# openclimatefix/graph_weather

Measured on AMD Instinct MI355X. Metric: forward forecasts/sec (1° grid, 102→78 feat), higher is better.
Workload: dtype f32; 1 GPU; c2: GraphWeatherForecaster 1deg grid (64800 nodes), 102->78 feat, batch=2 on rank 0, fp32, mesh res 2 (5882 nodes), random-init weights; global_batch=2, parallelism=batch-sharded x1, no collective in forward

## Files before the change

graph_weather_amd/csrc/gw_internal.hpp:

```cpp
#ifndef GW_INTERNAL_HPP
#define GW_INTERNAL_HPP

#include <hip/hip_runtime_api.h>
#include <stdint.h>

#include "../../include/gw_amd.h"

namespace gw {

enum { EPI_ROWS = 0, EPI_EDGE = 1, EPI_DEC = 2 };

struct ChainArgs {
  int n_cols;
  int cols_per_batch;
  unsigned long long* dbg;
  int dbg_cap;
  int stagger;
  const float* seg_ptr[3];
  const int* seg_idx[3];
  int seg_rows_pb[3];
  int seg_ld[3];
  int seg_k[3];
  int seg_proj[3];
  int seg_half[3];
  int seg_bf16k[3];
  const float* proj_w[4];
  float* proj_out[4];
  int n_post;
  const float* hd_w1;
  const float* hd_b1;
  const float* hd_w2;
  const float* hd_b2;
  const float* hd_w3;
  const float* hd_b3;
  int tune16;
  int proj_half;
  const float* w1[3];
  const float* b1;
  const float* w_mid;
  const float* b_mid;
  const float* w_out;
  const float* b_out;
  const float* gamma;
  const float* beta;
  int n_mid;
  const float* res_ptr;
  const int* res_idx;
  int res_rows_pb;
  int res_ld;
  float* out;
  int out_ld;
  int out_cols;
  int ln_width;
  float* agg;
  const int* agg_idx;
  int agg_rows_pb;
  const float* relu_mask;
  float* zero_rows;
  float* carry;
  float* save_h;
  long long save_stride;
  int save_ld;
  float* save_y;
};

int chain16_launch(int kind, ChainArgs& a, int k_in, int hidden, int n_out, int grid_y, void* stream);
int chainx3_launch(int kind, ChainArgs& a, int k_in, int hidden, int n_out, int grid_y, void* stream);
struct BwdChainArgs {
  const float* d;
  const void* w[5];
  const float* mask[2];
  float* out[5];
  long long n_rows;
  int d_ld, n_chain, n_fan;
  const float* ln_y;
  const float* ln_gamma;
  float* ln_dgamma;
  float* ln_dbeta;
  float* ln_dy;
  const float* add[5];
  int add_ld;
  float* colsum;
  const int* d_idx;
  int d_idx_n, d_tab_rows_pb;
  const float* d_add;
  int d_add_ld;
  unsigned add_d_mask;
};
int bwd_chainx3_launch(const BwdChainArgs& a, void* stream);
void pack_x3_item(const float* w, long long stride_f, long long stride_k, int n_out, int kseg, int ntp, int nsteps, void* out, void* stream);

int node_rs_groups(int64_t n_cols);
bool node_rs_eligible(const ChainArgs& a);
int node_rs_launch(ChainArgs& a, bool x3 , void* stream);

extern unsigned long long* g_dbg;
extern int g_dbg_cap;
extern int g_dbg_kind;
#ifdef GW_TUNING
int env_int(const char* name, int fallback);
#define GW_TUNE(name, fallback) gw::env_int(name, fallback)
#define GW_SKIP(a) ((a).skip)
#define GW_TUNE_ARG(a) ((a).tune)
#else
#define GW_TUNE(name, fallback) (fallback)
#define GW_SKIP(a) 0
#define GW_TUNE_ARG(a) 0
#endif

struct DeviceOnce {
  bool done[64] = {};
  bool first() {
    int d = 0;
    if (hipGetDevice(&d) != hipSuccess || d < 0 || d >= 64) return true;
    if (done[d]) return false;
    done[d] = true;
    return true;
  }
};
int set_error(int code, const char* msg);
int check_launch(const char* what);

constexpr int kCarryFloats = 528;
size_t segment_carry_bytes(int64_t n_tiles);
int segment_fixup_launch(int64_t n_tiles, const float* carry, float* agg, void* stream);

bool edge_fast_eligible(const gw_operand* x_src, const gw_operand* x_dst, const gw_operand* e_in, const gw_mlp_weights* w);
int edge_fast_launch(int32_t batch, int32_t n_edges, const int32_t* src, const int32_t* dst, const gw_operand* x_src,
                     const gw_operand* x_dst, const gw_operand* e_in, const gw_operand* e_res, const gw_mlp_weights* w,
                     float* e_out, float* agg, int32_t n_dst, const gw_activation_save* save, float* carry ,
                     void* stream);
size_t edge_fast_carry_bytes(int32_t batch, int32_t n_edges);

bool edge_stream_eligible(const gw_operand* x_src, const gw_operand* x_dst, const gw_operand* e_in, const gw_mlp_weights* w);
int edge_stream_launch(int32_t batch, int32_t n_edges, const int32_t* src, const int32_t* dst, const gw_operand* x_src,
                       const gw_operand* x_dst, const gw_operand* e_in, const gw_mlp_weights* w, float* agg, int32_t n_dst,
                       void* stream);

bool edge16_eligible(const gw_operand* x_src, const gw_operand* x_dst, const gw_operand* e_in, const gw_mlp_weights* w);
size_t edge16_workspace_bytes(int32_t batch, int32_t n_edges);
int edge16_launch(int32_t batch, int32_t n_edges, const int32_t* src, const int32_t* dst, const gw_operand* x_src,
                  const gw_operand* x_dst, const gw_operand* e_in, const gw_operand* e_res, const gw_mlp_weights* w,
                  float* e_out, void* e_out_tiles, float* agg, int32_t n_dst, void* workspace, int32_t flags ,
                  void* stream);
size_t edge16_workspace_needed(int32_t batch, int32_t n_edges, const gw_operand* e_in, bool deterministic);
int edge16t_launch(const void* edge16_args , bool gather, int n_wg, void* stream);
int edge16p_launch(const void* edge16_args , int n_wg, void* stream);
int edge16_rows_to_tiles(int32_t batch, int32_t n_edges, const float* rows, int32_t rows_per_batch, int32_t ld, void* tiles,
                         void* stream);

int ln_bwd_wide_launch(int64_t rows, int32_t width, const float* dn, int32_t ld_dn, const float* y, int32_t ld_y, const float* gamma,
                       float* dy, int32_t ld_dy, float* dgamma, float* dbeta, void* stream);
int relu_mask_wide_launch(int64_t rows, int32_t width, const float* dh, int32_t ld_dh, const float* h, int32_t ld_h, float* dz,
                          int32_t ld_dz, float* db, void* stream);

}

#endif
```

graph_weather_amd/csrc/gw_kernels.hip:

```cpp

#include <hip/hip_runtime.h>
#include <stdint.h>
#include <stdio.h>
#include <stdlib.h>
#include <string.h>

#include "../../include/gw_amd.h"
#include "gw_device.hpp"
#include "gw_internal.hpp"

using namespace gw;

namespace {

template <int NSTEPS>
__device__ __forceinline__ void load_operand_slice(float (&in)[NSTEPS], const float* __restrict__ row, int c, int q) {
#pragma unroll
  for (int i = 2 * c; i < 2 * c + 2; ++i) {
    if (4 * i + 3 < NSTEPS) {
      const f32x4 v = ldg4(row + 16 * i + 4 * q);
      in[4 * i + 0] = v.x;
      in[4 * i + 1] = v.y;
      in[4 * i + 2] = v.z;
      in[4 * i + 3] = v.w;
// ... 927 lines not shown
    if (a.bf16) {
      a.nsteps[i] = m.kseg <= 32 ? 1 : (m.kseg <= 128 ? 4 : (m.kseg + 31) / 32);
      a.ntq[i] = (nt + 3) / 4 * 4;
    } else {
      a.nsteps[i] = packed_steps_f32(m.kseg);
      a.ntq[i] = (nt + 3) / 4;
    }
  }
  for (int i = 0; i < n_vecs; ++i) {
    if (!vecs[i].v || !vecs[i].out || vecs[i].n <= 0) return fail(GW_E_BADARG, "gw_pack_many: bad vector item");
    a.v[i] = vecs[i];
  }
  hipLaunchKernelGGL(pack_many_kernel, dim3(64, n_mats + (n_vecs > 0 ? 1 : 0)), dim3(256), 0, (hipStream_t)stream, a);
  return check_launch("pack_many_kernel launch");
}

namespace {
int fill_bwd_chain(BwdChainArgs& a, int64_t n_rows, const float* d, int32_t d_ld, int32_t n_chain, const void* const* chain_w,
                   const float* const* chain_mask, float* const* chain_out, int32_t n_fan, const void* const* fan_w, float* const* fan_out) {
  if (n_rows < 0 || !d || d_ld < 256 || d_ld % 4 != 0 || n_chain < 0 || n_chain > 2 || n_fan < 0 || n_fan > 3 || n_chain + n_fan < 1 ||
      (n_chain > 0 && (!chain_w || !chain_mask || !chain_out)) || (n_fan > 0 && (!fan_w || !fan_out)))
    return fail(GW_E_BADARG, "gw_mlp_chain_backward: bad arguments");
  memset(&a, 0, sizeof(a));
  a.d = d;
  a.d_ld = d_ld;
  a.n_rows = n_rows;
  a.n_chain = n_chain;
  a.n_fan = n_fan;
  for (int i = 0; i < n_chain; ++i) {
    if (!chain_w[i] || !chain_mask[i] || !chain_out[i]) return fail(GW_E_BADARG, "gw_mlp_chain_backward: NULL chain item");
    a.w[i] = chain_w[i];
    a.mask[i] = chain_mask[i];
    a.out[i] = chain_out[i];
  }
  for (int i = 0; i < n_fan; ++i) {
    if (!fan_w[i] || !fan_out[i]) return fail(GW_E_BADARG, "gw_mlp_chain_backward: NULL fan item");
    a.w[n_chain + i] = fan_w[i];
    a.out[n_chain + i] = fan_out[i];
  }
  if ((n_rows + kColsPerWG - 1) / kColsPerWG > 0x7fffffffLL) return fail(GW_E_BADARG, "gw_mlp_chain_backward: too many rows");
  return GW_OK;
}
}

int gw_mlp_chain_backward(int64_t n_rows, const float* d, int32_t d_ld, int32_t n_chain, const float* const* chain_w,
                          const float* const* chain_mask, float* const* chain_out, int32_t n_fan, const float* const* fan_w,
                          float* const* fan_out, void* stream) {
  BwdChainArgs a;
  if (int rc = fill_bwd_chain(a, n_rows, d, d_ld, n_chain, (const void* const*)chain_w, chain_mask, chain_out, n_fan, (const void* const*)fan_w,
                              fan_out))
    return rc;
  if (n_rows == 0) return GW_OK;
  return bwd_chain_launch(a, stream);
}

int gw_mlp_ln_chain_backward(int32_t weight_dtype, int64_t n_rows, const float* dn, int32_t dn_ld, const int32_t* dn_idx,
                             int32_t dn_idx_n, int32_t dn_table_rows_pb, const float* dn_add, int32_t dn_add_ld, const float* y,
                             const float* gamma, float* dgamma, float* dbeta, float* dy, int32_t n_chain, const void* const* chain_w,
                             const float* const* chain_mask, float* const* chain_out, float* dz_colsum, int32_t n_fan,
                             const void* const* fan_w, float* const* fan_out, const float* const* fan_add, int32_t fan_add_ld,
                             uint32_t fan_add_dn_mask, void* stream) {
  const bool ln = y != nullptr;
  if (ln && (!gamma || !dgamma || !dbeta || !dy)) return fail(GW_E_BADARG, "gw_mlp_ln_chain_backward: NULL LayerNorm argument");
  if (weight_dtype != GW_DTYPE_BF16X3 && weight_dtype != GW_DTYPE_F32)
    return fail(GW_E_UNSUPPORTED, "gw_mlp_ln_chain_backward: fp32 or split (GW_DTYPE_BF16X3) streams");
  if (dz_colsum && n_chain < 1) return fail(GW_E_BADARG, "gw_mlp_ln_chain_backward: dz_colsum needs a chain product");
  if (fan_add && (fan_add_ld < 256 || fan_add_ld % 4 != 0)) return fail(GW_E_BADARG, "gw_mlp_ln_chain_backward: bad fan_add_ld");
  if ((dn_idx || dn_add) && !ln) return fail(GW_E_UNSUPPORTED, "gw_mlp_ln_chain_backward: a gathered input gradient needs the LayerNorm in front");
  if (dn_add && !dn_idx) return fail(GW_E_BADARG, "gw_mlp_ln_chain_backward: dn_add goes with dn_idx");
  if (dn_idx && (dn_idx_n <= 0 || dn_table_rows_pb <= 0 || n_rows % dn_idx_n != 0 || (dn_add && (dn_add_ld < 256 || dn_add_ld % 4 != 0))))
    return fail(GW_E_BADARG, "gw_mlp_ln_chain_backward: bad gather arguments");
  if (fan_add_dn_mask >> (n_fan > 0 ? n_fan : 0)) return fail(GW_E_BADARG, "gw_mlp_ln_chain_backward: fan_add_dn_mask names a fan item that does not exist");
  BwdChainArgs a;
  if (int rc = fill_bwd_chain(a, n_rows, dn, dn_ld, n_chain, chain_w, chain_mask, chain_out, n_fan, fan_w, fan_out)) return rc;
  if (n_rows == 0) return GW_OK;
  if (ln) {
    a.ln_y = y;
    a.ln_gamma = gamma;
    a.ln_dgamma = dgamma;
    a.ln_dbeta = dbeta;
    a.ln_dy = dy;
  }
  a.d_idx = dn_idx;
  a.d_idx_n = dn_idx_n;
  a.d_tab_rows_pb = dn_table_rows_pb;
  a.d_add = dn_add;
  a.d_add_ld = dn_add_ld;
  a.colsum = dz_colsum;
  a.add_ld = fan_add_ld;
  for (int i = 0; fan_add && i < n_fan; ++i) a.add[n_chain + i] = fan_add[i];
  a.add_d_mask = fan_add_dn_mask << n_chain;
  return weight_dtype == GW_DTYPE_BF16X3 ? bwd_chainx3_launch(a, stream) : bwd_chain_launch(a, stream);
}

int gw_mlp_chain_backward_bf16x3(int64_t n_rows, const float* d, int32_t d_ld, int32_t n_chain, const void* const* chain_w,
                                 const float* const* chain_mask, float* const* chain_out, int32_t n_fan, const void* const* fan_w,
                                 float* const* fan_out, void* stream) {
  BwdChainArgs a;
  if (int rc = fill_bwd_chain(a, n_rows, d, d_ld, n_chain, chain_w, chain_mask, chain_out, n_fan, fan_w, fan_out)) return rc;
  if (n_rows == 0) return GW_OK;
  return bwd_chainx3_launch(a, stream);
}

int gw_pad_vector(const float* v, int n, float* out, void* stream) {
  if (!v || !out || n <= 0) return fail(GW_E_BADARG, "gw_pad_vector: bad arguments");
  const int npad = gw_padded_n(n);
  hipLaunchKernelGGL(pad_vector_kernel, dim3((npad + 255) / 256), dim3(256), 0, (hipStream_t)stream, v, n, npad, out);
  return check_launch("pad_vector_kernel launch");
}

namespace {
int fill_save(ChainArgs& a, const gw_activation_save* save, const gw_mlp_weights* w, const char* who) {
  if (!save) return GW_OK;
  if (w->weight_dtype == GW_DTYPE_BF16)
    return fail(GW_E_UNSUPPORTED, "activation saving (training) is implemented for fp32 and bf16x3 weights (the saves are fp32 rows)");
  if (!save->hidden || save->hidden_ld < w->hidden || save->hidden_ld % 4 != 0 || (w->ln_gamma && !save->pre_norm)) {
    snprintf(g_err, sizeof(g_err), "%s: bad gw_activation_save", who);
    return GW_E_BADARG;
  }
  a.save_h = save->hidden;
  a.save_stride = save->hidden_stride;
  a.save_ld = save->hidden_ld;
  a.save_y = save->pre_norm;
  return GW_OK;
}
}

int gw_mlp_forward(int64_t n_rows, int32_t rows_per_batch, const gw_operand* x, const gw_mlp_weights* w,
                   const gw_operand* residual, float* out, int32_t out_ld, const gw_activation_save* save, void* stream) {
  if (!x || !w || !out || n_rows < 0 || rows_per_batch <= 0) return fail(GW_E_BADARG, "gw_mlp_forward: bad arguments");
  if (n_rows == 0) return GW_OK;
  if (n_rows >= (int64_t)1 << 31) return fail(GW_E_UNSUPPORTED, "gw_mlp_forward: more than 2^31-1 rows");
  if (x->k <= 0 || !w->w1[0] || !w->w_out || !w->b1 || !w->b_out)
    return fail(GW_E_BADARG, "gw_mlp_forward: missing weights / empty operand");
  if (x->layout != GW_LAYOUT_ROWS_F32 || (residual && residual->layout != GW_LAYOUT_ROWS_F32))
    return fail(GW_E_UNSUPPORTED, "gw_mlp_forward: operands are fp32 rows");
  if (bad_layers(w)) return fail(GW_E_UNSUPPORTED, "gw_mlp_forward: at least 2 hidden layers (n_mid >= 1) are required");
  ChainArgs a;
  memset(&a, 0, sizeof(a));
  a.n_cols = (int)n_rows;
  a.cols_per_batch = rows_per_batch;
  fill_operand(a, 0, x);
  fill_weights(a, w);
  if (residual) {
    a.res_ptr = residual->ptr;
    a.res_idx = residual->index;
    a.res_rows_pb = residual->rows_per_batch;
    a.res_ld = residual->ld;
  }
  a.out = out;
  a.out_ld = out_ld;
  a.out_cols = w->n_out;
  if (int rc = fill_save(a, save, w, "gw_mlp_forward")) return rc;
  if (is16(w->weight_dtype)) {
    if (residual && w->n_out == 256 && (residual->ld % 4 != 0)) return fail(GW_E_UNSUPPORTED, "gw_mlp_forward: residual ld must be a multiple of 4");
    if (w->n_out == 256 && out_ld % 4 != 0) return fail(GW_E_UNSUPPORTED, "gw_mlp_forward: out_ld must be a multiple of 4");
    if (x->k == 256 && x->ld % 4 != 0) return fail(GW_E_UNSUPPORTED, "gw_mlp_forward: input ld must be a multiple of 4");
    if (x->k > 128 && x->k != 256) return fail(GW_E_UNSUPPORTED, "gw_mlp_forward: input width must be <=128 or ==256");
    if (w->weight_dtype == GW_DTYPE_BF16 && w->ln_gamma && (w->n_out != 256 || (w->ln_width > 0 && w->ln_width != w->n_out)))
      return fail(GW_E_UNSUPPORTED, "gw_mlp_forward: LayerNorm over fewer than 256 features is implemented for float32 and bf16x3 weights");
    return launch16(w->weight_dtype, 0, a, x->k, w->hidden, w->n_out, 1, stream);
  }
  if (w->hidden == 256 && w->n_out == 256) {
    if (residual && (residual->ld % 4 != 0)) return fail(GW_E_UNSUPPORTED, "gw_mlp_forward: residual ld must be a multiple of 4");
    if (out_ld % 4 != 0) return fail(GW_E_UNSUPPORTED, "gw_mlp_forward: out_ld must be a multiple of 4");
    if (x->k <= 16) return launch_chain(chain_kernel<4, false, 1, 16, 16, EPI_ROWS>, a, stream);
    if (x->k <= 112) return launch_chain(chain_kernel<28, false, 1, 16, 16, EPI_ROWS>, a, stream);
    if (x->k == 256 && x->ld % 4 == 0) return launch_chain(chain_kernel<64, true, 1, 16, 16, EPI_ROWS>, a, stream);
    return fail(GW_E_UNSUPPORTED, "gw_mlp_forward: input width must be <=112 or ==256 for hidden 256");
  }
  if (w->hidden == 256 && w->n_out <= 80 && x->k == 256 && x->ld % 4 == 0) {
    return launch_chain(chain_kernel<64, true, 1, 16, 5, EPI_DEC>, a, stream);
  }
  if (w->hidden == 128 && w->n_out <= 80 && x->k == 256 && x->ld % 4 == 0) {
    return launch_chain(chain_kernel<64, true, 1, 8, 5, EPI_DEC>, a, stream);
  }
  return fail(GW_E_UNSUPPORTED, "gw_mlp_forward: unsupported (hidden, n_out, k) combination");
}

int gw_mlp_post_forward(int64_t n_rows, int32_t rows_per_batch, const gw_operand* x, const gw_mlp_weights* w, float* out,
                        int32_t out_ld, int32_t n_post, const float* const* post_w, void* const* post_out, int32_t post_layout,
                        void* stream) {
  if (!x || !w || n_rows < 0 || rows_per_batch <= 0 || n_post <= 0 || n_post > 4 || !post_w || !post_out)
    return fail(GW_E_BADARG, "gw_mlp_post_forward: bad arguments");
  if (n_rows == 0) return GW_OK;
  if (n_rows >= (int64_t)1 << 31) return fail(GW_E_UNSUPPORTED, "gw_mlp_post_forward: more than 2^31-1 rows");
  if (x->k <= 0 || !w->w1[0] || !w->w_out || !w->b1 || !w->b_out) return fail(GW_E_BADARG, "gw_mlp_post_forward: missing weights / empty operand");
  if (x->layout != GW_LAYOUT_ROWS_F32) return fail(GW_E_UNSUPPORTED, "gw_mlp_post_forward: x is fp32 rows");
  if (bad_layers(w)) return fail(GW_E_UNSUPPORTED, "gw_mlp_post_forward: at least 2 hidden layers (n_mid >= 1) are required");
  if (!is16(w->weight_dtype) || w->hidden != 256 || w->n_out != 256 || !w->ln_gamma || (w->ln_width > 0 && w->ln_width != 256))
    return fail(GW_E_UNSUPPORTED, "gw_mlp_post_forward: bf16 / bf16x3 weights, hidden 256, 256 outputs with LayerNorm");
  if (post_layout != GW_LAYOUT_ROWS_F32 && post_layout != GW_LAYOUT_ROWS_F16) return fail(GW_E_BADARG, "gw_mlp_post_forward: bad post_layout");
  if (post_layout == GW_LAYOUT_ROWS_F16 && w->weight_dtype != GW_DTYPE_BF16)
    return fail(GW_E_UNSUPPORTED, "gw_mlp_post_forward: fp16 products come with bf16 weights");
  if (out && out_ld % 4 != 0) return fail(GW_E_UNSUPPORTED, "gw_mlp_post_forward: out_ld must be a multiple of 4");
  ChainArgs a;
  memset(&a, 0, sizeof(a));
  a.n_cols = (int)n_rows;
  a.cols_per_batch = rows_per_batch;
  fill_operand(a, 0, x);
  fill_weights(a, w);
  a.out = out;
  a.out_ld = out ? out_ld : 256;
  a.out_cols = 256;
  for (int i = 0; i < n_post; ++i) {
    if (!post_w[i] || !post_out[i]) return fail(GW_E_BADARG, "gw_mlp_post_forward: null post slice / output");
    a.proj_w[i] = post_w[i];
    a.proj_out[i] = (float*)post_out[i];
  }
  a.n_post = n_post;
  a.proj_half = post_layout == GW_LAYOUT_ROWS_F16;
  return launch16(w->weight_dtype, 5, a, x->k, w->hidden, w->n_out, 1, stream);
}

size_t gw_edge_update_workspace_bytes(int32_t batch, int32_t n_edges, const gw_operand* x_src, const gw_operand* x_dst,
                                      const gw_operand* e_in, const gw_mlp_weights* w, int32_t flags) {
  if (batch <= 0 || n_edges <= 0 || !x_src || !x_dst || !e_in || !w) return 0;
  const bool det = (flags & GW_EDGE_DETERMINISTIC) != 0;
  if (gw::edge16_eligible(x_src, x_dst, e_in, w)) return gw::edge16_workspace_needed(batch, n_edges, e_in, det);
  if (det && w->weight_dtype == GW_DTYPE_F32 && gw::edge_fast_eligible(x_src, x_dst, e_in, w)) return gw::edge_fast_carry_bytes(batch, n_edges);
  if (det && is16(w->weight_dtype)) return gw::edge_fast_carry_bytes(batch, n_edges);
  return 0;
}

size_t gw_edge_tiles_bytes(int32_t batch, int32_t n_edges) {
  if (batch <= 0 || n_edges <= 0) return 0;
  return gw::edge16_workspace_bytes(batch, n_edges);
}

int gw_edge_rows_to_tiles(int32_t batch, int32_t n_edges, const float* rows, int32_t rows_per_batch, int32_t ld, void* tiles,
                          void* stream) {
  if (batch <= 0 || n_edges <= 0 || !rows || !tiles || ld < 256 || ld % 4 != 0 || rows_per_batch < 0)
    return fail(GW_E_BADARG, "gw_edge_rows_to_tiles: bad arguments");
  return gw::edge16_rows_to_tiles(batch, n_edges, rows, rows_per_batch, ld, tiles, stream);
}

int gw_edge_update_forward(int32_t batch, int32_t n_edges, const int32_t* src, const int32_t* dst,
                           const gw_operand* x_src, const gw_operand* x_dst, const gw_operand* e_in,
                           const gw_operand* e_res, const gw_mlp_weights* w, void* e_out_any, int32_t e_out_layout, float* agg,
                           int32_t n_dst, const gw_activation_save* save, void* workspace, size_t workspace_bytes, int32_t flags,
                           void* stream) {
  if (batch <= 0 || n_edges < 0 || n_dst <= 0) return fail(GW_E_BADARG, "gw_edge_update_forward: bad arguments");
  if (n_edges == 0) return GW_OK;
  if (!src || !dst || !x_src || !x_dst || !e_in || !e_res || !w || !agg) return fail(GW_E_BADARG, "gw_edge_update_forward: bad arguments");
  if ((int64_t)batch * n_edges >= (int64_t)1 << 31 || (int64_t)batch * n_dst >= (int64_t)1 << 31)
    return fail(GW_E_UNSUPPORTED, "gw_edge_update_forward: batch*edges exceeds int32");
  if (w->hidden != 256 || w->n_out != 256 || (w->ln_gamma == nullptr) != (w->ln_beta == nullptr) || !w->b1 || !w->w_out || !w->b_out)
    return fail(GW_E_UNSUPPORTED, "gw_edge_update_forward: only hidden=256, out=256 is implemented");
  if (bad_layers(w)) return fail(GW_E_UNSUPPORTED, "gw_edge_update_forward: at least 2 hidden layers (n_mid >= 1) are required");
  const gw_operand* ops[3] = {x_src, x_dst, e_in};
  for (int i = 0; i < 3; ++i) {
    if (ops[i]->k == 0) continue;
    if (ops[i]->k != 256 || ops[i]->ld % 4 != 0 || !ops[i]->ptr || (!ops[i]->projected && !w->w1[i]))
      return fail(GW_E_UNSUPPORTED, "gw_edge_update_forward: operands must be 256 wide (or k=0 for zeros)");
  }
  const bool no_res = e_res->k == 0;
  const bool x3 = w->weight_dtype == GW_DTYPE_BF16X3;
  const bool stream32 = no_res && !(flags & (GW_EDGE_DETERMINISTIC | GW_EDGE_SEGMENT_TILES)) && gw::edge_stream_eligible(x_src, x_dst, e_in, w);
  if (no_res && (e_out_any != nullptr || save || !(x3 || stream32 || (gw::edge16_eligible(x_src, x_dst, e_in, w) && !(flags & GW_EDGE_DETERMINISTIC)))))
    return fail(GW_E_UNSUPPORTED, "gw_edge_update_forward: an edge update without residual (e_res.k == 0) is implemented for the bf16 "
                                  "path with resident weights (atomics mode), for bf16x3 weights and for float32 weights with projected "
                                  "operands only (one middle layer, LayerNorm over 256, atomics mode), without e_out or activation saving");
  if (!no_res && (e_res->k != 256 || e_res->ld % 4 != 0 || !e_res->ptr))
    return fail(GW_E_UNSUPPORTED, "gw_edge_update_forward: e_res (residual edge features) must be 256 wide");
  const bool tiles_in = (e_in->k > 0 && e_in->layout == GW_LAYOUT_EDGE_TILES_BF16) || e_res->layout == GW_LAYOUT_EDGE_TILES_BF16;
  const bool tiles_out = e_out_any != nullptr && e_out_layout == GW_LAYOUT_EDGE_TILES_BF16;
  if (e_out_any != nullptr && e_out_layout != GW_LAYOUT_ROWS_F32 && e_out_layout != GW_LAYOUT_EDGE_TILES_BF16)
    return fail(GW_E_BADARG, "gw_edge_update_forward: bad e_out_layout");
  if ((e_in->k > 0 && e_in->layout != GW_LAYOUT_ROWS_F32 && e_in->layout != GW_LAYOUT_EDGE_TILES_BF16) ||
      (!no_res && e_res->layout != GW_LAYOUT_ROWS_F32 && e_res->layout != GW_LAYOUT_EDGE_TILES_BF16))
    return fail(GW_E_UNSUPPORTED, "gw_edge_update_forward: edge operands are fp32 rows or bf16 edge tiles");
  const bool half_nodes = x_src->layout == GW_LAYOUT_ROWS_F16 || x_dst->layout == GW_LAYOUT_ROWS_F16;
  if ((x_src->layout != GW_LAYOUT_ROWS_F32 && x_src->layout != GW_LAYOUT_ROWS_F16) ||
      (x_dst->layout != GW_LAYOUT_ROWS_F32 && x_dst->layout != GW_LAYOUT_ROWS_F16) ||
      (half_nodes && (save || !gw::edge16_eligible(x_src, x_dst, e_in, w))))
    return fail(GW_E_UNSUPPORTED, "gw_edge_update_forward: node operands must be fp32 rows (or, projected, for the bf16 path with "
                                  "resident weights: fp16 product rows)");
  float* e_out = tiles_out ? nullptr : (float*)e_out_any;
  const bool det = (flags & GW_EDGE_DETERMINISTIC) != 0;
  const bool seg = (flags & GW_EDGE_SEGMENT_TILES) != 0;
  if ((flags & (GW_EDGE_AGG_BF16K | GW_EDGE_SEGMENT_SPLIT)) && !seg)
    return fail(GW_E_BADARG, "gw_edge_update_forward: GW_EDGE_AGG_BF16K / GW_EDGE_SEGMENT_SPLIT come with GW_EDGE_SEGMENT_TILES");
  if (seg) {
    const size_t ws_seg = gw::edge16_eligible(x_src, x_dst, e_in, w) ? gw::edge16_workspace_needed(batch, n_edges, e_in, false) : 0;
    if (det || save || n_edges % 64 != 0 || !gw::edge16_eligible(x_src, x_dst, e_in, w) || (e_out_any && !tiles_out) ||
        (!no_res && e_res->layout != GW_LAYOUT_EDGE_TILES_BF16) || (ws_seg > 0 && (!workspace || workspace_bytes < ws_seg)))
      return fail(GW_E_UNSUPPORTED, "gw_edge_update_forward: segment-aligned tiles (GW_EDGE_SEGMENT_TILES) are implemented for the bf16 "
                                    "path with resident weights: projected node operands, residual none or bf16 edge tiles, e' none "
                                    "or bf16 edge tiles, atomics mode, n_edges a multiple of 64, the workspace of "
                                    "gw_edge_update_workspace_bytes");
    return gw::edge16_launch(batch, n_edges, src, dst, x_src, x_dst, e_in, e_res, w, nullptr, tiles_out ? e_out_any : nullptr, agg, n_dst,
                             workspace, flags, stream);
  }
  if (stream32) return gw::edge_stream_launch(batch, n_edges, src, dst, x_src, x_dst, e_in, w, agg, n_dst, stream);
  const size_t ws16 = gw::edge16_workspace_needed(batch, n_edges, e_in, det);
  if (det && save) return fail(GW_E_UNSUPPORTED, "gw_edge_update_forward: deterministic segment sums are an inference option");
  if (tiles_in || tiles_out || (no_res && !x3) || half_nodes) {
    if (save || (ws16 > 0 && (!workspace || workspace_bytes < ws16)) || !gw::edge16_eligible(x_src, x_dst, e_in, w))
      return fail(GW_E_UNSUPPORTED, "gw_edge_update_forward: bf16 edge tiles need bf16 weights, one middle layer, projected node "
                                    "operands, no activation saving and the workspace of gw_edge_update_workspace_bytes");
    return gw::edge16_launch(batch, n_edges, src, dst, x_src, x_dst, e_in, e_res, w, e_out, tiles_out ? e_out_any : nullptr, agg,
                             n_dst, workspace, det ? GW_EDGE_DETERMINISTIC : 0, stream);
  }
  if (w->weight_dtype == GW_DTYPE_F32 && (!save || w->n_mid == 1) && gw::edge_fast_eligible(x_src, x_dst, e_in, w)) {
    if (save && (!save->hidden || !save->pre_norm || save->hidden_ld < 256 || save->hidden_ld % 4 != 0))
      return fail(GW_E_BADARG, "gw_edge_update_forward: bad gw_activation_save");
    if (det && (!workspace || workspace_bytes < gw::edge_fast_carry_bytes(batch, n_edges)))
      return fail(GW_E_BADARG, "gw_edge_update_forward: deterministic mode needs the workspace of gw_edge_update_workspace_bytes");
    return gw::edge_fast_launch(batch, n_edges, src, dst, x_src, x_dst, e_in, e_res, w, e_out, agg, n_dst, save,
                                det ? (float*)workspace : nullptr, stream);
  }
  if (!save && gw::edge16_eligible(x_src, x_dst, e_in, w) && (ws16 == 0 || (workspace && workspace_bytes >= ws16)))
    return gw::edge16_launch(batch, n_edges, src, dst, x_src, x_dst, e_in, e_res, w, e_out, nullptr, agg, n_dst, workspace,
                             det ? GW_EDGE_DETERMINISTIC : 0, stream);
  if (det && (!is16(w->weight_dtype) || !workspace || workspace_bytes < gw::edge_fast_carry_bytes(batch, n_edges)))
    return fail(GW_E_UNSUPPORTED, "gw_edge_update_forward: deterministic segment sums exist on the fast fp32 edge kernel (at most one "
                                  "raw operand, native 256 widths) and on the bf16 kernels, and need their workspace");
  ChainArgs a;
  memset(&a, 0, sizeof(a));
  a.n_cols = batch * n_edges;
  a.cols_per_batch = n_edges;
  fill_operand(a, 0, x_src);
  a.seg_idx[0] = src;
  fill_operand(a, 1, x_dst);
  a.seg_idx[1] = dst;
  fill_operand(a, 2, e_in);
  fill_weights(a, w);
  if (!no_res) fill_residual(a, e_res);
  a.out = e_out;
  a.out_ld = 256;
  a.out_cols = 256;
  a.agg = agg;
  a.agg_idx = dst;
  a.agg_rows_pb = n_dst;
  if (int rc = fill_save(a, save, w, "gw_edge_update_forward")) return rc;
  if (is16(w->weight_dtype)) {
    if (w->weight_dtype == GW_DTYPE_BF16 && w->ln_gamma && a.ln_width != 256)
      return fail(GW_E_UNSUPPORTED, "gw_edge_update_forward: LayerNorm over fewer than 256 features needs float32 or bf16x3 weights");
    if (det) a.carry = (float*)workspace;
    if (int rc = launch16(w->weight_dtype, 1, a, 256, 256, 256, 1, stream)) return rc;
    return det ? gw::segment_fixup_launch(((int64_t)a.n_cols + 63) / 64, a.carry, agg, stream) : GW_OK;
  }
  return launch_chain(chain_kernel<64, true, 3, 16, 16, EPI_EDGE>, a, stream, 1, 1);
}

int gw_node_update_forward(int64_t n_rows, int32_t rows_per_batch, const gw_operand* x, const gw_operand* x_res,
                           const gw_operand* agg, const gw_mlp_weights* w, float* x_out, int32_t out_ld,
                           const gw_activation_save* save, int32_t n_post, const float* const* post_w, void* const* post_out,
                           int32_t post_layout, float* zero_rows, void* stream) {
  if (!x || !agg || !w || !x_out || n_rows < 0 || rows_per_batch <= 0) return fail(GW_E_BADARG, "gw_node_update_forward: bad arguments");
  if (n_rows == 0) return GW_OK;
  if (n_rows >= (int64_t)1 << 31) return fail(GW_E_UNSUPPORTED, "gw_node_update_forward: more than 2^31-1 rows");
  if (w->hidden != 256 || w->n_out != 256 || !w->b1 || !w->w_out || !w->b_out)
    return fail(GW_E_UNSUPPORTED, "gw_node_update_forward: only hidden=256, out=256");
  if (bad_layers(w)) return fail(GW_E_UNSUPPORTED, "gw_node_update_forward: at least 2 hidden layers (n_mid >= 1) are required");
  if (bad_agg(agg, w->weight_dtype == GW_DTYPE_BF16) || !w->w1[1])
    return fail(GW_E_UNSUPPORTED, "gw_node_update_forward: agg must be 256 wide (raw fp32 rows; bf16 rows in K order with bf16 weights)");
  if (agg->layout == GW_LAYOUT_ROWS_BF16K && save) return fail(GW_E_UNSUPPORTED, "gw_node_update_forward: bf16 aggregates are an inference format");
  if (x->k != 0 && (bad256(x, w->weight_dtype == GW_DTYPE_BF16) || (!x->projected && !w->w1[0])))
    return fail(GW_E_UNSUPPORTED, "gw_node_update_forward: x must be 256 wide (fp32 rows; fp16 product rows with bf16 weights) or zeros");
  if (x_res && x_res->k != 0 && bad256(x_res)) return fail(GW_E_UNSUPPORTED, "gw_node_update_forward: x_res must be 256 wide");
  if (out_ld % 4 != 0) return fail(GW_E_UNSUPPORTED, "gw_node_update_forward: out_ld must be a multiple of 4");
  ChainArgs a;
  memset(&a, 0, sizeof(a));
  a.n_cols = (int)n_rows;
  a.cols_per_batch = rows_per_batch;
  fill_operand(a, 0, x);
  fill_operand(a, 1, agg);
  fill_weights(a, w);
  if (x_res && x_res->k != 0) fill_residual(a, x_res);
  a.out = x_out;
  a.out_ld = out_ld;
  a.out_cols = 256;
  if (int rc = fill_save(a, save, w, "gw_node_update_forward")) return rc;
  if (n_post < 0 || n_post > 4 || (n_post > 0 && (!post_w || !post_out))) return fail(GW_E_BADARG, "gw_node_update_forward: bad post products");
  if ((n_post > 0 || zero_rows) && (save || out_ld != 256)) return fail(GW_E_UNSUPPORTED, "gw_node_update_forward: post products need out_ld 256, no activation saving");
  if (zero_rows && n_post == 0) return fail(GW_E_BADARG, "gw_node_update_forward: zero_rows comes with post products");
  for (int i = 0; i < n_post; ++i) {
    if (!post_w[i] || !post_out[i]) return fail(GW_E_BADARG, "gw_node_update_forward: null post slice / output");
    a.proj_w[i] = post_w[i];
    a.proj_out[i] = (float*)post_out[i];
  }
  a.n_post = n_post;
  if (post_layout != GW_LAYOUT_ROWS_F32 && post_layout != GW_LAYOUT_ROWS_F16) return fail(GW_E_BADARG, "gw_node_update_forward: bad post_layout");
  if (post_layout == GW_LAYOUT_ROWS_F16 && (n_post == 0 || w->weight_dtype != GW_DTYPE_BF16))
    return fail(GW_E_UNSUPPORTED, "gw_node_update_forward: fp16 post products come with bf16 weights");
  a.proj_half = post_layout == GW_LAYOUT_ROWS_F16;
  a.zero_rows = zero_rows;
  if (w->weight_dtype != GW_DTYPE_BF16 && GW_TUNE("GW_NODE_RS", 1) != 0 && gw::node_rs_eligible(a))
    return gw::node_rs_launch(a, w->weight_dtype == GW_DTYPE_BF16X3, stream);
  if (is16(w->weight_dtype)) {
    if (w->weight_dtype == GW_DTYPE_BF16 && w->ln_gamma && a.ln_width != 256)
      return fail(GW_E_UNSUPPORTED, "gw_node_update_forward: LayerNorm over fewer than 256 features needs float32 or bf16x3 weights");
    return launch16(w->weight_dtype, n_post > 0 ? 4 : 2, a, 256, 256, 256, 1, stream);
  }
  if (n_post > 0) return launch_chain(chain_kernel<64, true, 2, 16, 16, EPI_ROWS, false, true>, a, stream, 1, 2);
  return launch_chain(chain_kernel<64, true, 2, 16, 16, EPI_ROWS>, a, stream, 1, 2);
}

int gw_node_update_row_split_groups(int64_t n_rows) { return gw::node_rs_groups(n_rows); }

int gw_node_update_head_forward(int64_t n_rows, int32_t rows_per_batch, const gw_operand* x, const gw_operand* agg,
                                const gw_mlp_weights* w, const gw_mlp_weights* head, const gw_operand* residual, float* out,
                                int32_t out_ld, void* stream) {
  if (!x || !agg || !w || !head || !out || n_rows < 0 || rows_per_batch <= 0) return fail(GW_E_BADARG, "gw_node_update_head_forward: bad arguments");
  if (n_rows == 0) return GW_OK;
  if (n_rows >= (int64_t)1 << 31) return fail(GW_E_UNSUPPORTED, "gw_node_update_head_forward: more than 2^31-1 rows");
  if (head->weight_dtype != w->weight_dtype)
    return fail(GW_E_UNSUPPORTED, "gw_node_update_head_forward: the same weight dtype for both MLPs");
  const bool b16 = w->weight_dtype == GW_DTYPE_BF16;
  if (w->hidden != 256 || w->n_out != 256 || !w->b1 || !w->w_out || !w->b_out || bad_layers(w) || w->n_mid != 1 || !w->ln_gamma ||
      (w->ln_width > 0 && w->ln_width != 256))
    return fail(GW_E_UNSUPPORTED, "gw_node_update_head_forward: node MLP must be 512 -> 256 -> 256 -> 256 with LayerNorm");
  if (bad_agg(agg, b16) || !w->w1[1]) return fail(GW_E_UNSUPPORTED, "gw_node_update_head_forward: agg must be 256 wide (raw)");
  if (x->k != 0 && (bad256(x, b16) || (!x->projected && !w->w1[0]))) return fail(GW_E_UNSUPPORTED, "gw_node_update_head_forward: x must be 256 wide or zeros");
  if (head->hidden != 128 || head->n_mid != 1 || head->n_out > 80 || head->n_out <= 0 || head->ln_gamma || !head->w1[0] || !head->b1 ||
      !head->w_mid || !head->b_mid || !head->w_out || !head->b_out)
    return fail(GW_E_UNSUPPORTED, "gw_node_update_head_forward: the head must be 256 -> 128 -> 128 -> <= 80 features without norm");
  if (head->k_in != 256 || (head->out_rows != 80 && !(head->out_rows == 0 && head->n_out == 80)))
    return fail(GW_E_UNSUPPORTED, "gw_node_update_head_forward: the head must be packed for 256 inputs (k_in) and 80 output rows (out_rows)");
  ChainArgs a;
  memset(&a, 0, sizeof(a));
  a.n_cols = (int)n_rows;
  a.cols_per_batch = rows_per_batch;
  fill_operand(a, 0, x);
  fill_operand(a, 1, agg);
  fill_weights(a, w);
  a.hd_w1 = head->w1[0];
  a.hd_b1 = head->b1;
  a.hd_w2 = head->w_mid;
  a.hd_b2 = head->b_mid;
  a.hd_w3 = head->w_out;
  a.hd_b3 = head->b_out;
  if (residual && residual->k != 0) {
    if (!residual->ptr || residual->layout != GW_LAYOUT_ROWS_F32) return fail(GW_E_BADARG, "gw_node_update_head_forward: bad residual");
    fill_residual(a, residual);
  }
  a.out = out;
  a.out_ld = out_ld;
  a.out_cols = head->n_out;
  if (!is16(w->weight_dtype)) {
    if (x->k != 0 && x->layout != GW_LAYOUT_ROWS_F32) return fail(GW_E_UNSUPPORTED, "gw_node_update_head_forward: fp32 weights take fp32 rows");
    return launch_chain(chain_kernel<64, true, 2, 16, 16, EPI_ROWS, false, false, true>, a, stream, 1, 2);
  }
  return launch16(w->weight_dtype, 6, a, 256, 256, 256, 1, stream);
}

int gw_project_forward(int64_t n_rows, int32_t rows_per_batch, const gw_operand* x, int32_t n_slices,
                       const float* const* w_slices, void* const* outs, int32_t out_ld, int32_t out_layout, int32_t weight_dtype,
                       const float* relu_mask, float* zero_rows, void* stream) {
  if (!x || !w_slices || !outs || n_rows < 0 || rows_per_batch <= 0 || n_slices <= 0 || n_slices > 4)
    return fail(GW_E_BADARG, "gw_project_forward: bad arguments (1..4 slices)");
  if (n_rows == 0) return GW_OK;
  if (n_rows >= (int64_t)1 << 31) return fail(GW_E_UNSUPPORTED, "gw_project_forward: more than 2^31-1 rows");
  if (bad256(x) || x->projected || out_ld % 4 != 0) return fail(GW_E_UNSUPPORTED, "gw_project_forward: x must be a raw 256-wide table");
  ChainArgs a;
  memset(&a, 0, sizeof(a));
  a.n_cols = (int)n_rows;
  a.cols_per_batch = rows_per_batch;
  fill_operand(a, 0, x);
  for (int i = 0; i < n_slices; ++i) {
    if (!w_slices[i] || !outs[i]) return fail(GW_E_BADARG, "gw_project_forward: null slice / output");
    a.proj_w[i] = w_slices[i];
    a.proj_out[i] = (float*)outs[i];
  }
  if (out_layout != GW_LAYOUT_ROWS_F32 && out_layout != GW_LAYOUT_ROWS_F16) return fail(GW_E_BADARG, "gw_project_forward: bad out_layout");
  if (out_layout == GW_LAYOUT_ROWS_F16 && weight_dtype != GW_DTYPE_BF16)
    return fail(GW_E_UNSUPPORTED, "gw_project_forward: fp16 products come with bf16 slices");
  a.proj_half = out_layout == GW_LAYOUT_ROWS_F16;
  a.out_ld = out_ld;
  a.out_cols = 256;
  if (relu_mask && (weight_dtype == GW_DTYPE_BF16 || n_slices != 1))
    return fail(GW_E_UNSUPPORTED, "gw_project_forward: relu_mask needs fp32 or bf16x3 weights and a single slice");
  a.relu_mask = relu_mask;
  if (zero_rows && weight_dtype != GW_DTYPE_F32) return fail(GW_E_UNSUPPORTED, "gw_project_forward: zero_rows needs fp32 weights");
  a.zero_rows = zero_rows;
  if (is16(weight_dtype)) return launch16(weight_dtype, 3, a, 256, 256, 256, n_slices, stream);
  return launch_chain(chain_kernel<64, true, 1, 16, 16, EPI_ROWS, true>, a, stream, n_slices, 3);
}

int gw_normalized_mse_forward(const float* pred, const float* target, const float* inv_var, int32_t inv_var_full,
                              const float* lat_weights, int32_t num_unique_lat, int32_t batch, int32_t nodes, int32_t channels,
                              float* loss_out, void* stream) {
  if (!pred || !target || !lat_weights || !loss_out || num_unique_lat <= 0 || batch <= 0 || nodes <= 0 || channels <= 0)
    return fail(GW_E_BADARG, "gw_normalized_mse_forward: bad arguments");
  const int num_lon = nodes / num_unique_lat;
  if (num_lon <= 0 || (nodes + num_lon - 1) / num_lon > num_unique_lat)
    return fail(GW_E_BADARG, "gw_normalized_mse_forward: nodes must equal num_unique_lat * num_lon");
  const size_t total = (size_t)batch * nodes * channels;
  const float scale = 1.0f / ((float)channels * (float)batch * (float)nodes);
  int grid = (int)((total + 1023) / 1024);
  if (grid > 2048) grid = 2048;
  hipLaunchKernelGGL(nmse_kernel, dim3(grid), dim3(256), 0, (hipStream_t)stream, pred, target, inv_var, inv_var_full, lat_weights, num_lon, nodes,
                     channels, total, scale, loss_out);
  return check_launch("nmse_kernel launch");
}

}
```

Before: 310.0 forecasts/s.

## Add LDS-staged fp32 edge MLP kernel with pipelined operand gathers

```diff
diff --git a/graph_weather_amd/csrc/gw_edge_lds.hip b/graph_weather_amd/csrc/gw_edge_lds.hip
--- /dev/null
+++ b/graph_weather_amd/csrc/gw_edge_lds.hip
@@ -0,0 +1,461 @@
+
+#include <hip/hip_runtime.h>
+#include <stdint.h>
+#include <string.h>
+
+#include "gw_device.hpp"
+#include "gw_edge_common.hpp"
+#include "gw_internal.hpp"
+
+using namespace gw;
+
+namespace {
+
+constexpr int kConstFloats = 5 * 256;
+constexpr int kConstOff = kStageFloats + kColsPerWG;
+constexpr int kEldsLdsBytes = (kConstOff + kConstFloats) * 4;
+static_assert(kEldsLdsBytes == 71936, "staging + destination ids + constants");
+static_assert((kConstOff * 4) % 16 == 0, "constants are read as 16-byte vectors");
+static_assert(2 * kEldsLdsBytes <= 160 * 1024, "two workgroups per CU must fit the 160 KiB of LDS");
+constexpr int kB1 = 0, kBMid = 256, kBOut = 512, kGamma = 768, kBeta = 1024;
+
+struct EldsArgs {
+  int n_cols;
+  int n_edges;
+  int n_dst;
+  int stagger;
+  int skip;
+  int dma6;
+  int xcd_base;
+  int xcd_rem;
+  const int* src;
+  const int* dst;
+  const float* raw_ptr;
+  int raw_rows_pb;
+  int raw_ld;
+  int raw_kind;
+  const float* w_raw;
+  const float* p_ptr[3];
+  int p_rows_pb[3];
+  int p_ld[3];
+  int p_kind[3];
+  const float* b1;
+  const float* w_mid;
+  const float* b_mid;
+  const float* w_out;
+  const float* b_out;
+  const float* gamma;
+  const float* beta;
+  const float* res_ptr;
+  int res_rows_pb;
+  int res_ld;
+  float* e_out;
+  float* agg;
+};
+
+template <bool RAW>
+__device__ __forceinline__ const float* chunk_src(const EldsArgs& a, int i) {
+  if (RAW) {
+    if (i < kChunksPerLayer) return a.w_raw + (size_t)i * kChunkFloats;
+    i -= kChunksPerLayer;
+  }
+  if (i < kChunksPerLayer) return a.w_mid + (size_t)i * kChunkFloats;
+  return a.w_out + (size_t)(i - kChunksPerLayer) * kChunkFloats;
+}
+
+__device__ __forceinline__ float hld1(const float* p) {
+  float v;
+  asm volatile("global_load_dword %0, %1, off" : "=v"(v) : "v"(p) : "memory");
+  return v;
+}
+template <int N>
+__device__ __forceinline__ void wait_prologue(int& s, int& d, float (&c)[5]) {
+  asm volatile("s_waitcnt vmcnt(%[n])" : "+v"(s), "+v"(d), "+v"(c[0]), "+v"(c[1]), "+v"(c[2]), "+v"(c[3]), "+v"(c[4]) : [n] "n"(N) : "memory");
+}
+
+template <bool RAW, int NPROJ>
+__global__ __launch_bounds__(kThreads, 2) void elds_kernel(const EldsArgs a) {
+  float* const lds = lds_base();
+  const float* const cst = lds + kConstOff;
+  const int lane = threadIdx.x & 63;
+  const int wave = __builtin_amdgcn_readfirstlane(threadIdx.x >> 6);
+  const int j = lane & 15;
+  const int q = lane >> 4;
+  int tile = blockIdx.x;
+  if (a.xcd_base > 0) {
+    const int xcd = tile & 7, idx = tile >> 3;
+    tile = xcd * a.xcd_base + (xcd < a.xcd_rem ? xcd : a.xcd_rem) + idx;
+  }
+  const int tile_c0 = tile * kColsPerWG;
+  const int c_raw = tile_c0 + wave * kColsPerWave + j;
+  const bool valid = c_raw < a.n_cols;
+  const int c = valid ? c_raw : a.n_cols - 1;
+  const int b = c / a.n_edges;
+  const int k = c - b * a.n_edges;
+
+  if (a.stagger > 0 && (blockIdx.x >> 8) == 1) {
+    for (int i = 0; i < a.stagger; ++i) __builtin_amdgcn_s_sleep(127);
+  }
+
+  int s_idx = hldi(a.src + k);
+  int d_idx = hldi(a.dst + k);
+  float cv[5];
+  {
+    const int f = threadIdx.x;
+    cv[0] = hld1(a.b1 + f);
+    cv[1] = hld1(a.b_mid + f);
+    cv[2] = hld1(a.b_out + f);
+    cv[3] = hld1(a.gamma + f);
+    cv[4] = hld1(a.beta + f);
+  }
+  issue_chunk32k(chunk_src<RAW>(a, 0), lds, lane, wave);
+  int ci = 0;
+  wait_prologue<8>(s_idx, d_idx, cv);
+  {
+    float* cw = lds + kConstOff + threadIdx.x;
+    cw[kB1] = cv[0];
+    cw[kBMid] = cv[1];
+    cw[kBOut] = cv[2];
+    cw[kGamma] = cv[3];
+    cw[kBeta] = cv[4];
+  }
+
+  const float* prow[NPROJ];
+#pragma unroll
+  for (int p = 0; p < NPROJ; ++p) {
+    const int r = a.p_kind[p] == 0 ? s_idx : (a.p_kind[p] == 1 ? d_idx : k);
+    prow[p] = a.p_ptr[p] + ((size_t)b * (size_t)a.p_rows_pb[p] + (size_t)r) * (size_t)a.p_ld[p] + 4 * q;
+  }
+  const int gd_id = valid ? b * a.n_dst + d_idx : -1;
+
+  f32x4 ring[2][NPROJ][2];
+#define GW_REQUEST_SLICE(slot, slice)                                          \
+  {                                                                            \
+    _Pragma("unroll") for (int p = 0; p < NPROJ; ++p) {                        \
+      ring[slot][p][0] = hld4<128 * (slice)>(prow[p]);                         \
+      ring[slot][p][1] = hld4<128 * (slice) + 64>(prow[p]);                    \
+    }                                                                          \
+  }
+#define GW_BIAS_SLICE(slice)                                                   \
+  if (!RAW) {                                                                  \
+    bb0 = *(const f32x4*)(cst + kB1 + 32 * (slice) + 4 * q);                   \
+    bb1 = *(const f32x4*)(cst + kB1 + 32 * (slice) + 16 + 4 * q);              \
+  }
+#define GW_CONSUME_SLICE(slot, slice)                                          \
+  {                                                                            \
+    f32x4 v0_, v1_;                                                            \
+    if (RAW) {                                                                 \
+      v0_ = acc[2 * (slice)] + ring[slot][0][0];                               \
+      v1_ = acc[2 * (slice) + 1] + ring[slot][0][1];                           \
+    } else {                                                                   \
+      v0_ = ring[slot][0][0];                                                  \
+      v1_ = ring[slot][0][1];                                                  \
+    }                                                                          \
+    _Pragma("unroll") for (int p = 1; p < NPROJ; ++p) {                        \
+      v0_ += ring[slot][p][0];                                                 \
+      v1_ += ring[slot][p][1];                                                 \
+    }                                                                          \
+    if (!RAW) {                                                                \
+      v0_ += bb0;                                                              \
+      v1_ += bb1;                                                              \
+    }                                                                          \
+    _Pragma("unroll") for (int r = 0; r < 4; ++r) {                            \
+      in8[r] = fmaxf(v0_[r], 0.f);                                             \
+      in8[4 + r] = fmaxf(v1_[r], 0.f);                                         \
+    }                                                                          \
+  }
+
+  f32x4 a_cur[4];
+  f32x4 acc[16];
+  f32x4 acc2[16];
+  float in8[8];
+  f32x4 bb0, bb1;
+  if (RAW) {
+    const int r = a.raw_kind == 0 ? s_idx : (a.raw_kind == 1 ? d_idx : k);
+    const float* xrow = a.raw_ptr + ((size_t)b * (size_t)a.raw_rows_pb + (size_t)r) * (size_t)a.raw_ld + 4 * q;
+    f32x4 xv[16];
+    hld_row(xv, xrow);
+    wait_regs<0>(xv);
+    lds_barrier();
+#pragma unroll
+    for (int t = 0; t < 16; ++t) acc[t] = *(const f32x4*)(cst + kB1 + 16 * t + 4 * q);
+#pragma unroll
+    for (int b4 = 0; b4 < 4; ++b4) a_cur[b4] = *(const f32x4*)(lds + lane * 4 + b4 * 256);
+    float x[64];
+#pragma unroll
+    for (int i = 0; i < 16; ++i) {
+      x[4 * i + 0] = xv[i].x;
+      x[4 * i + 1] = xv[i].y;
+      x[4 * i + 2] = xv[i].z;
+      x[4 * i + 3] = xv[i].w;
+    }
+#pragma unroll
+    for (int cc = 0; cc < kChunksPerLayer; ++cc) {
+#pragma unroll
+      for (int i = 0; i < 8; ++i) in8[i] = x[8 * cc + i];
+      if (cc == kChunksPerLayer - 3) {
+        GW_REQUEST_SLICE(0, 0)
+        GW_REQUEST_SLICE(1, 1)
+      }
+      if (cc == kChunksPerLayer - 1) {
+#pragma unroll
+        for (int t = 0; t < 16; ++t) acc2[t] = *(const f32x4*)(cst + kBMid + 16 * t + 4 * q);
+      }
+      GW_CHUNK(acc, in8, true, wait_vm<0>(), chunk_src<RAW>(a, ci + 1))
+    }
+    wait_regs<0>(ring[0]);
+    wait_regs<0>(ring[1]);
+    GW_CONSUME_SLICE(0, 0)
+    GW_REQUEST_SLICE(0, 2)
+  } else {
+    GW_REQUEST_SLICE(0, 0)
+    GW_REQUEST_SLICE(1, 1)
+    wait_regs<2 * NPROJ>(ring[0]);
+    lds_barrier();
+#pragma unroll
+    for (int t = 0; t < 16; ++t) acc2[t] = *(const f32x4*)(cst + kBMid + 16 * t + 4 * q);
+    GW_BIAS_SLICE(0)
+#pragma unroll
+    for (int b4 = 0; b4 < 4; ++b4) a_cur[b4] = *(const f32x4*)(lds + lane * 4 + b4 * 256);
+    GW_CONSUME_SLICE(0, 0)
+    GW_REQUEST_SLICE(0, 2)
+  }
+
+#define GW_PRODUCE_CHUNK(cc)                                                              \
+  {                                                                                       \
+    if ((cc) + 1 < kChunksPerLayer) GW_BIAS_SLICE((cc) + 1)                                \
+    if ((cc) <= 6) {                                                                      \
+      GW_CHUNK(acc2, in8, true, wait_regs<0>(ring[((cc) + 1) & 1]), chunk_src<RAW>(a, ci + 1))                        \
+    } else {                                                                              \
+      GW_CHUNK(acc2, in8, true, wait_vm<0>(), chunk_src<RAW>(a, ci + 1))                                              \
+    }                                                                                     \
+    if ((cc) + 1 < kChunksPerLayer) GW_CONSUME_SLICE(((cc) + 1) & 1, (cc) + 1)             \
+  }
+  GW_PRODUCE_CHUNK(0)
+  GW_REQUEST_SLICE(1, 3)
+  GW_PRODUCE_CHUNK(1)
+  GW_REQUEST_SLICE(0, 4)
+  GW_PRODUCE_CHUNK(2)
+  GW_REQUEST_SLICE(1, 5)
+  GW_PRODUCE_CHUNK(3)
+  GW_REQUEST_SLICE(0, 6)
+  GW_PRODUCE_CHUNK(4)
+  GW_REQUEST_SLICE(1, 7)
+  GW_PRODUCE_CHUNK(5)
+  GW_PRODUCE_CHUNK(6)
+  GW_PRODUCE_CHUNK(7)
+
+  float hin[64];
+#pragma unroll
+  for (int t = 0; t < 16; ++t)
+#pragma unroll
+    for (int r = 0; r < 4; ++r) hin[4 * t + r] = fmaxf(acc2[t][r], 0.f);
+  f32x4 o[16];
+  f32x4 rres[16];
+#pragma unroll
+  for (int t = 0; t < 16; ++t) o[t] = f32x4{0.f, 0.f, 0.f, 0.f};
+#pragma unroll
+  for (int cc = 0; cc < kChunksPerLayer; ++cc) {
+#pragma unroll
+    for (int i = 0; i < 8; ++i) in8[i] = hin[8 * cc + i];
+    if (cc + 1 < kChunksPerLayer) {
+      GW_CHUNK(o, in8, true, wait_vm<0>(), chunk_src<RAW>(a, ci + 1))
+    } else {
+      GW_CHUNK(o, in8, false, wait_vm<0>(), chunk_src<RAW>(a, ci + 1))
+    }
+    if (cc == 3 || cc == 5) {
+      const float* rrow = a.res_ptr + ((size_t)b * (size_t)a.res_rows_pb + (size_t)k) * (size_t)a.res_ld + 4 * q;
+      if (cc == 3) hld_half_row<0>(rres, rrow); else hld_half_row<1>(rres, rrow);
+    }
+  }
+  wait_regs<0>(rres);
+
+  {
+#pragma unroll
+    for (int t = 0; t < 16; ++t) o[t] += *(const f32x4*)(cst + kBOut + 16 * t + 4 * q);
+    constexpr float inv_n = 1.0f / 256.0f;
+    float s = 0.f;
+#pragma unroll
+    for (int t = 0; t < 16; ++t) s += (o[t].x + o[t].y) + (o[t].z + o[t].w);
+    s += __shfl_xor(s, 16);
+    s += __shfl_xor(s, 32);
+    const float mean = s * inv_n;
+    float v = 0.f;
+#pragma unroll
+    for (int t = 0; t < 16; ++t)
+#pragma unroll
+      for (int r = 0; r < 4; ++r) {
+        const float d = o[t][r] - mean;
+        v += d * d;
+      }
+    v += __shfl_xor(v, 16);
+    v += __shfl_xor(v, 32);
+    const float rstd = 1.0f / sqrtf(v * inv_n + 1e-5f);
+#pragma unroll
+    for (int t = 0; t < 16; ++t) {
+      const f32x4 gm = *(const f32x4*)(cst + kGamma + 16 * t + 4 * q);
+      const f32x4 bt = *(const f32x4*)(cst + kBeta + 16 * t + 4 * q);
+#pragma unroll
+      for (int r = 0; r < 4; ++r) o[t][r] = (o[t][r] - mean) * rstd * gm[r] + bt[r] + rres[t][r];
+    }
+  }
+
+  __syncthreads();
+  {
+    float* srow = lds + (wave * kColsPerWave + j) * kStageLd + 4 * q;
+#pragma unroll
+    for (int t = 0; t < 16; ++t) *(f32x4*)(srow + 16 * t) = o[t];
+    if (q == 0) ((int*)(lds + kStageFloats))[wave * kColsPerWave + j] = gd_id;
+  }
+  __syncthreads();
+  const int* gdl = (const int*)(lds + kStageFloats);
+
+  if (a.e_out != nullptr) {
+#pragma unroll 4
+    for (int i = 0; i < kColsPerWave; ++i) {
+      const int col = wave * kColsPerWave + i;
+      if (tile_c0 + col < a.n_cols) {
+        const f32x4 vv = *(const f32x4*)(lds + col * kStageLd + 4 * lane);
+        stg4(a.e_out + (size_t)(tile_c0 + col) * 256 + 4 * lane, vv);
+      }
+    }
+  }
+
+  {
+    const int f = threadIdx.x;
+    float vv[kColsPerWG];
+#pragma unroll
+    for (int i = 0; i < kColsPerWG; ++i) vv[i] = lds[i * kStageLd + f];
+    const int gdv = gdl[lane];
+    const int gdn = gdl[lane < kColsPerWG - 1 ? lane + 1 : lane];
+    const unsigned long long ends = __ballot(lane == kColsPerWG - 1 || gdn != gdv);
+    float run = 0.f;
+    bool first = true;
+#pragma unroll
+    for (int i = 0; i < kColsPerWG; ++i) {
+      run += vv[i];
+      if (__builtin_expect((ends >> i) & 1ull, 0)) {
+        const int cur = __builtin_amdgcn_readlane(gdv, i);
+        if (cur >= 0) {
+          float* dstp = a.agg + (size_t)cur * 256 + f;
+          if (first || i == kColsPerWG - 1) {
+            __hip_atomic_fetch_add((GW_AS1 float*)dstp, run, __ATOMIC_RELAXED, __HIP_MEMORY_SCOPE_AGENT);
+          } else {
+            stg1(dstp, run);
+          }
+        }
+        first = false;
+        run = 0.f;
+      }
+    }
+  }
+#undef GW_REQUEST_SLICE
+#undef GW_BIAS_SLICE
+#undef GW_CONSUME_SLICE
+#undef GW_PRODUCE_CHUNK
+}
+
+template <typename K>
+int launch(K kernel, const EldsArgs& a, void* stream) {
+  static DeviceOnce once;
+  if (once.first()) (void)hipFuncSetAttribute((const void*)kernel, hipFuncAttributeMaxDynamicSharedMemorySize, kEldsLdsBytes);
+  const int grid = (a.n_cols + kColsPerWG - 1) / kColsPerWG;
+  hipLaunchKernelGGL(kernel, dim3(grid), dim3(kThreads), kEldsLdsBytes, (hipStream_t)stream, a);
+  return check_launch("elds_kernel launch");
+}
+
+inline bool f32_rows(const gw_operand* op) { return op->layout == GW_LAYOUT_ROWS_F32; }
+
+inline bool count_operands(const gw_operand* x_src, const gw_operand* x_dst, const gw_operand* e_in, int& n_raw, int& n_proj) {
+  const gw_operand* ops[3] = {x_src, x_dst, e_in};
+  n_raw = n_proj = 0;
+  for (int i = 0; i < 3; ++i) {
+    if (ops[i]->k == 0) continue;
+    if (!f32_rows(ops[i])) return false;
+    if (ops[i]->projected) ++n_proj; else ++n_raw;
+  }
+  return true;
+}
+
+}
+
+namespace gw {
+
+bool edge_lds_eligible(const gw_operand* x_src, const gw_operand* x_dst, const gw_operand* e_in, const gw_mlp_weights* w) {
+  if (w->weight_dtype != GW_DTYPE_F32 || w->n_mid != 1 || !w->ln_gamma || !w->ln_beta || !w->w_mid || !w->b_mid) return false;
+  if (w->ln_width > 0 && w->ln_width != 256) return false;
+  int n_raw, n_proj;
+  if (!count_operands(x_src, x_dst, e_in, n_raw, n_proj)) return false;
+  if (!(n_raw == 1 ? (n_proj == 1 || n_proj == 2) : (n_raw == 0 && n_proj == 3))) return false;
+  static const int impl = GW_TUNE("GW_EDGE_LDS", 1);
+  return impl != 0 && edge_fast_eligible(x_src, x_dst, e_in, w);
+}
+
+int edge_lds_launch(int32_t batch, int32_t n_edges, const int32_t* src, const int32_t* dst, const gw_operand* x_src,
+                    const gw_operand* x_dst, const gw_operand* e_in, const gw_operand* e_res, const gw_mlp_weights* w, float* e_out,
+                    float* agg, int32_t n_dst, void* stream) {
+  EldsArgs a;
+  memset(&a, 0, sizeof(a));
+  a.n_cols = batch * n_edges;
+  a.n_edges = n_edges;
+  a.n_dst = n_dst;
+  const int tiles = (a.n_cols + kColsPerWG - 1) / kColsPerWG;
+  a.src = src;
+  a.dst = dst;
+  const gw_operand* ops[3] = {x_src, x_dst, e_in};
+  int n_proj = 0, n_raw = 0;
+  for (int i = 0; i < 3; ++i) {
+    if (ops[i]->k == 0) continue;
+    if (!ops[i]->projected) {
+      if (n_raw == 1) return set_error(GW_E_UNSUPPORTED, "edge_lds_launch: at most one raw operand");
+      ++n_raw;
+      a.raw_ptr = ops[i]->ptr;
+      a.raw_rows_pb = ops[i]->rows_per_batch;
+      a.raw_ld = ops[i]->ld;
+      a.raw_kind = i;
+      a.w_raw = w->w1[i];
+    } else {
+      if (n_proj == 3) return set_error(GW_E_UNSUPPORTED, "edge_lds_launch: at most three projected operands");
+      a.p_ptr[n_proj] = ops[i]->ptr;
+      a.p_rows_pb[n_proj] = ops[i]->rows_per_batch;
+      a.p_ld[n_proj] = ops[i]->ld;
+      a.p_kind[n_proj] = i;
+      ++n_proj;
+    }
+  }
+  if (!(n_raw == 1 ? (n_proj == 1 || n_proj == 2) : n_proj == 3) || (n_raw == 1 && !a.w_raw))
+    return set_error(GW_E_UNSUPPORTED, "edge_lds_launch: one raw operand with one or two projected, or three projected operands");
+  a.b1 = w->b1;
+  a.w_mid = w->w_mid;
+  a.b_mid = w->b_mid;
+  a.w_out = w->w_out;
+  a.b_out = w->b_out;
+  a.gamma = w->ln_gamma;
+  a.beta = w->ln_beta;
+  a.res_ptr = e_res->ptr;
+  a.res_rows_pb = e_res->rows_per_batch;
+  a.res_ld = e_res->ld;
+  a.e_out = e_out;
+  a.agg = agg;
+  {
+    static const int skip = GW_TUNE("GW_EDGE_SKIP", 0);
+    static const int dma6 = GW_TUNE("GW_EDGE_DMA6", 0);
+    a.skip = skip == 4 || skip == 5 ? skip : 0;
+    a.dma6 = dma6;
+  }
+  {
+    static const int stagger_override = GW_TUNE("GW_STAGGER", -1);
+    const int passes = 2 + n_raw;
+    a.stagger = stagger_override >= 0 ? stagger_override * passes : 2 * passes + 2;
+    if (tiles <= 256) a.stagger = 0;
+  }
+  {
+    static const int xcd_map = GW_TUNE("GW_XCD_MAP", 1);
+    a.xcd_base = (xcd_map != 0 && tiles >= 64) ? tiles / 8 : 0;
+    a.xcd_rem = tiles % 8;
+  }
+  if (n_raw == 1) return n_proj == 1 ? launch(elds_kernel<true, 1>, a, stream) : launch(elds_kernel<true, 2>, a, stream);
+  return launch(elds_kernel<false, 3>, a, stream);
+}
+
+}
diff --git a/graph_weather_amd/csrc/gw_internal.hpp b/graph_weather_amd/csrc/gw_internal.hpp
--- a/graph_weather_amd/csrc/gw_internal.hpp
+++ b/graph_weather_amd/csrc/gw_internal.hpp
@@ -137,6 +137,11 @@
                        const gw_operand* x_dst, const gw_operand* e_in, const gw_mlp_weights* w, float* agg, int32_t n_dst,
                        void* stream);
 
+bool edge_lds_eligible(const gw_operand* x_src, const gw_operand* x_dst, const gw_operand* e_in, const gw_mlp_weights* w);
+int edge_lds_launch(int32_t batch, int32_t n_edges, const int32_t* src, const int32_t* dst, const gw_operand* x_src,
+                    const gw_operand* x_dst, const gw_operand* e_in, const gw_operand* e_res, const gw_mlp_weights* w, float* e_out,
+                    float* agg, int32_t n_dst, void* stream);
+
 bool edge16_eligible(const gw_operand* x_src, const gw_operand* x_dst, const gw_operand* e_in, const gw_mlp_weights* w);
 size_t edge16_workspace_bytes(int32_t batch, int32_t n_edges);
 int edge16_launch(int32_t batch, int32_t n_edges, const int32_t* src, const int32_t* dst, const gw_operand* x_src,
diff --git a/graph_weather_amd/csrc/gw_kernels.hip b/graph_weather_amd/csrc/gw_kernels.hip
--- a/graph_weather_amd/csrc/gw_kernels.hip
+++ b/graph_weather_amd/csrc/gw_kernels.hip
@@ -1253,6 +1253,8 @@
     return gw::edge16_launch(batch, n_edges, src, dst, x_src, x_dst, e_in, e_res, w, e_out, tiles_out ? e_out_any : nullptr, agg,
                              n_dst, workspace, det ? GW_EDGE_DETERMINISTIC : 0, stream);
   }
+  if (!save && !det && !seg && !no_res && e_res->layout == GW_LAYOUT_ROWS_F32 && gw::edge_lds_eligible(x_src, x_dst, e_in, w))
+    return gw::edge_lds_launch(batch, n_edges, src, dst, x_src, x_dst, e_in, e_res, w, e_out, agg, n_dst, stream);
   if (w->weight_dtype == GW_DTYPE_F32 && (!save || w->n_mid == 1) && gw::edge_fast_eligible(x_src, x_dst, e_in, w)) {
     if (save && (!save->hidden || !save->pre_norm || save->hidden_ld < 256 || save->hidden_ld % 4 != 0))
       return fail(GW_E_BADARG, "gw_edge_update_forward: bad gw_activation_save");
```

Result: faster. 314.3 forecasts/s, median of 6 (+1.4%).
